# williamyang1991/VToonify

Hardware: AMD Instinct MI355X
Metric: frames/sec at 1024x1024 VToonify-D inference (higher is better)
Workload: dtype bf16

## Files before the change

### vtoonify_amd/csrc/conv_igemm.hip

```cpp
#include <stdlib.h>
#include <utility>

#include "vt_common.hpp"

namespace {

#ifdef VT_EMU
typedef emu_f32x4 f32x4;
#else
typedef float f32x4 __attribute__((ext_vector_type(4)));
typedef __bf16 bf16x8_t __attribute__((ext_vector_type(8)));
#endif

static inline int slab_ld(int cout_total) { return (cout_total + 31) / 32 * 32; }
constexpr int64_t VT_TICKET_BYTES = 16384;

struct ConvArgs {
    const void* src0;
    const void* src1;
    const void* wgt;
    const float* bias;
    const float* slope_vec;
    const void* rgb_w;
    const float* rgb_bias;
// ... 1378 lines not shown
        }
        if (rgbf && p.rgb_resid) {
#pragma unroll
            for (int j = 0; j < 3; ++j) rsd[j] = p.rgb_resid[o_rgb + (int64_t)j * HoWo];
        }
        f32x4 acc[TM][TN];
#pragma unroll
        for (int a = 0; a < TM; ++a)
#pragma unroll
            for (int b = 0; b < TN; ++b) acc[a][b] = f32x4{0.f, 0.f, 0.f, 0.f};
        const unsigned char* sa = smem + buf * A_BYTES;
#pragma unroll
        for (int t = 0; t < 9; ++t) {
            const int ky = t / 3, kx = t - ky * 3;
            u128 fa[TM];
#pragma unroll
            for (int a = 0; a < TM; ++a) {
                const int pr = (wm * TM + a + ky) * PW + kx + l15;
                fa[a] = ld128(sa + pr * 64 + ((q ^ swz(pr)) << 4));
            }
#pragma unroll
            for (int a = 0; a < TM; ++a)
#pragma unroll
                for (int b = 0; b < TN; ++b) Mma<T>::run(acc[a][b], wreg[t][b], fa[a]);
            vt_sched_fence();
        }
        {
            const float ga = p.gain_alpha;
            f32x4 racc = f32x4{0.f, 0.f, 0.f, 0.f};
#pragma unroll
            for (int a = 0; a < TM; ++a) {
                const int m = rowmap(wm * (TM * 16) + a * 16 + l15);
                float f[8];
#pragma unroll
                for (int b = 0; b < TN; ++b) {
#pragma unroll
                    for (int i = 0; i < 4; ++i) {
                        float v = acc[a][b][i] + bvr[b][i];
                        if (p.act == VT_ACT_LRELU) v = (v > 0.0f) ? v : v * p.slope;
                        f[4 * b + i] = v * ga;
                    }
                }
                const u128 fpk = pack16<bf16_t>(f);
                if (rgbf) {
                    const bool mine = (l15 >> 2) == a;
                    u128 wa;
                    wa.x = mine ? rwf.x : 0u, wa.y = mine ? rwf.y : 0u, wa.z = mine ? rwf.z : 0u, wa.w = mine ? rwf.w : 0u;
                    Mma<bf16_t>::run(racc, wa, fpk);
                }
                if (m >= 0 && !p.rgb_only) st128((bf16_t*)p.out + (int64_t)m * p.ld_out + cg + q * 8, fpk);
            }
            if (rgbf) {
                const float rr[3] = {racc[0], racc[1], racc[2]};
                if (m_rgb >= 0) {
                    p.rgb_out[o_rgb] = rr[0] + rb0 + rsd[0];
                    p.rgb_out[o_rgb + HoWo] = rr[1] + rb1 + rsd[1];
                    p.rgb_out[o_rgb + 2 * (int64_t)HoWo] = rr[2] + rb2 + rsd[2];
                }
            }
        }
        vt_lds_barrier();
        buf = buf + 1 == NBUF ? 0 : buf + 1;
    }
}

template <int... I, typename F>
__device__ __forceinline__ void vt_static_for_impl(std::integer_sequence<int, I...>, F&& f) {
    (f(std::integral_constant<int, I>{}), ...);
}
template <int N, typename F>
__device__ __forceinline__ void vt_static_for(F&& f) {
    vt_static_for_impl(std::make_integer_sequence<int, N>{}, static_cast<F&&>(f));
}

#include "conv_fullk.hpp"
#include "conv_fullkw.hpp"
#include "conv_upblur.hpp"
static int device_cus();
#include "conv_upblur_rows.hpp"
#include "conv_upblur_flat.hpp"
#include "conv_thin.hpp"
#include "conv_patch_pipe.hpp"
#include "conv_patch_chunk.hpp"
#include "conv_patch_s2.hpp"
#include "conv_patch_resident.hpp"
#include "conv_patch_persist.hpp"

__device__ __forceinline__ int slab_col4(const ConvArgs& p, int n) {
    return p.slab_perm ? (n & ~31) + ((n >> 2) & 1) * 16 + ((n >> 3) & 3) * 4 : n;
}

__global__ void __launch_bounds__(256) conv_splitk_reduce_kernel(const ConvArgs p) {
    const int nv = p.ldp / 8;
    const int64_t total = (int64_t)p.M * nv;
    const int64_t slab = (int64_t)p.M * p.ldp;
    const float ga = p.gain_alpha * (p.alpha_dev ? p.alpha_dev[0] : 1.0f);
    const int HoWo = p.Ho * p.Wo;
    for (int64_t idx = (int64_t)blockIdx.x * 256 + threadIdx.x; idx < total; idx += (int64_t)gridDim.x * 256) {
        int m, v8;
        if (p.out_layout == VT_OUT_NHWC) {
            m = (int)(idx / nv);
            v8 = (int)(idx - (int64_t)m * nv);
        } else {
            v8 = (int)(idx / p.M);
            m = (int)(idx - (int64_t)v8 * p.M);
        }
        const int n = v8 * 8;
        if (n >= p.coutT) continue;
        const int c0 = slab_col4(p, n);
        const int dc = slab_col4(p, n + 4) - c0;
        const float* src = p.partial + (int64_t)m * p.ldp + c0;
        float f[8];
        unpack16<float>(ld128(src), f);
        unpack16<float>(ld128(src + dc), f + 4);
        constexpr int SG = 8;
        for (int s0 = 1; s0 < p.splitk; s0 += SG) {
            float g[SG][8];
#pragma unroll
            for (int k = 0; k < SG; ++k) {
                const int s = (s0 + k < p.splitk) ? s0 + k : 0;
                unpack16<float>(ld128(src + s * slab), g[k]);
                unpack16<float>(ld128(src + s * slab + dc), g[k] + 4);
            }
#pragma unroll
            for (int k = 0; k < SG; ++k) {
                if (s0 + k < p.splitk) {
#pragma unroll
                    for (int i = 0; i < 8; ++i) f[i] += g[k][i];
                }
            }
        }
        {
            float bv8[8], sv8[8];
            int co8[8];
#pragma unroll
            for (int i = 0; i < 8; ++i) {
                const int nc = (n + i < p.coutT) ? n + i : 0;
                co8[i] = (p.phases > 1) ? nc % p.cout : nc;
                bv8[i] = 0.0f;
                sv8[i] = p.slope;
            }
            if (p.bias) {
#pragma unroll
                for (int i = 0; i < 8; ++i) bv8[i] = p.bias[co8[i]];
            }
            if (p.slope_vec) {
#pragma unroll
                for (int i = 0; i < 8; ++i) sv8[i] = p.slope_vec[co8[i]];
            }
#pragma unroll
            for (int i = 0; i < 8; ++i) {
                const bool okc = n + i < p.coutT;
                f[i] = conv_finish(p, f[i], okc ? bv8[i] : 0.0f, ga, okc ? sv8[i] : p.slope);
            }
        }
        if (p.out_layout == VT_OUT_NHWC) {
            store_nhwc8(p, m, n, f);
        } else {
            float* o = (float*)p.out;
            const float* rs = (const float*)p.resid;
            const int img = m / HoWo;
            const int rem = m - img * HoWo;
            for (int i = 0; i < 8 && n + i < p.coutT; ++i) {
                const int64_t off = ((int64_t)img * p.cout + n + i) * HoWo + rem;
                o[off] = post_act(p, f[i] + (rs ? p.beta * rs[off] : 0.0f));
            }
// ... 131 lines not shown
    constexpr int ESZ = (int)sizeof(T);
    constexpr int BK = 8 * (16 / ESZ);
    if (a.force_generic || a.transposed || a.in_scale) return false;
    if (a.c0 % BK != 0 || a.c1 % BK != 0) return false;
    const int64_t lim = ((int64_t)1 << 31) - 4096;
    const int64_t px = (int64_t)a.N * a.H * a.W;
    const int64_t b0 = ((int64_t)a.pad * a.W + a.pad) * a.ld0 * ESZ;
    const int64_t b1 = ((int64_t)a.pad * a.W + a.pad) * a.ld1 * ESZ;
    const int64_t n0 = px * a.ld0 * ESZ + b0, n1 = px * a.ld1 * ESZ + b1;
    const int64_t nw = (int64_t)a.coutT * a.K * ESZ;
    const int64_t tapmax = ((int64_t)(a.taps / a.kw - 1) * a.dil * a.W + (int64_t)(a.kw - 1) * a.dil);
    if (n0 + tapmax * a.ld0 * ESZ >= lim || n1 + tapmax * a.ld1 * ESZ >= lim || nw >= lim) return false;
    g.nrec0 = (uint32_t)n0;
    g.nrec1 = (uint32_t)n1;
    g.nrecw = (uint32_t)nw;
    g.bias0 = (uint32_t)b0;
    g.bias1 = (uint32_t)b1;
    return true;
}

static bool in_launch_rule(const ConvArgs& a, int64_t ntile) {
    if (a.phase != 0 || ntile * 4 > VT_TICKET_BYTES) return false;
    const char* e = getenv("VT_SPLITK_IN_LAUNCH");
    return e && e[0] == '1';
}
static void split_mode(ConvArgs& args) {
    if (args.splitk <= 1 || !in_launch_rule(args, (int64_t)args.tiles_m * args.tiles_n)) args.tickets = nullptr;
}

template <typename T, int BM, int BN, int WM, int WN>
int launch_cfg(const ConvArgs& a, vt_stream stream) {
    constexpr int BK = 8 * (16 / (int)sizeof(T));
    ConvArgs args = a;
    args.slab_perm = ((BN / WN / 16) % 2 == 0) ? 1 : 0;
    args.tiles_n = vt_cdiv(a.coutT, BN);
    args.tiles_m = vt_cdiv(a.M, BM);
    const int nk = vt_cdiv(a.K, BK);
    if (args.splitk > 1) {
        args.kps = vt_cdiv(nk, args.splitk);
        args.splitk = vt_cdiv(nk, args.kps);
    }
    if (args.splitk <= 1) {
        args.splitk = 1;
        args.kps = nk;
    }
    split_mode(args);
    const int64_t tiles = (int64_t)vt_cdiv(a.M, BM) * args.tiles_n * args.splitk;
    if (tiles >= ((int64_t)1 << 31)) {
        vt_set_error("vt_conv2d: too many tiles");
        return VT_ERR_ARG;
    }
    GldsArgs g;
    if (args.phase == 2) {
    } else if (glds_eligible<T>(args, g)) {
        if (args.splitk == 1 && args.tiles_n > 1 &&
            (int64_t)a.N * a.H * a.W * a.cin > (int64_t)a.coutT * a.K)
            args.blk_pm = -1;
        constexpr int STAGE = ((BM + 31) / 32 + (BN + 31) / 32) * 32 * 128;
        constexpr int NST = STAGE * 4 <= 80 * 1024 ? 4 : STAGE * 3 <= 80 * 1024 ? 3 : 2;
        bool done = false;
        if constexpr (sizeof(T) == 4 && !is_x3<T>::value) {
            if (a.x3) {
                auto k = conv_igemm_glds_kernel<f32x3_t, BM, BN, WM, WN, NST>;
                VT_LAUNCH(k, dim3((unsigned)tiles), dim3(256), stream, args, g);
                done = true;
            }
        }
        if (!done) {
            auto k = conv_igemm_glds_kernel<T, BM, BN, WM, WN, NST>;
            VT_LAUNCH(k, dim3((unsigned)tiles), dim3(256), stream, args, g);
        }
    } else {
        auto k = conv_igemm_kernel<T, BM, BN, WM, WN>;
        VT_LAUNCH(k, dim3((unsigned)tiles), dim3(256), stream, args);
    }
    int rc = vt_check_launch("vt_conv2d");
    if (rc != VT_OK || args.splitk == 1 || args.tickets || args.phase == 1) return rc;
    return launch_reduce<T>(args, stream);
}

struct TilePlan {
    int kind;
    int bm, bn, splitk;
};

template <typename T>
static bool patch_eligible(const ConvArgs& a, GldsArgs& g) {
    constexpr int ESZ = (int)sizeof(T);
    constexpr int BK = 8 * (16 / ESZ);
    if (a.force_generic || a.transposed || a.in_scale) return false;
    if (a.taps != 9 || a.kw != 3 || a.stride != 1 || a.pad != a.dil) return false;
    if (a.dil != 1 && a.dil != 2 && a.dil != 4) return false;
    if (a.Ho != a.H || a.Wo != a.W) return false;
    if (a.c0 % BK != 0 || a.c1 % BK != 0) return false;
    const int64_t lim = ((int64_t)1 << 31) - 4096;
    const int64_t px = (int64_t)a.N * a.H * a.W;
    const int64_t n0 = px * a.ld0 * ESZ, n1 = px * a.ld1 * ESZ, nw = (int64_t)a.coutT * a.K * ESZ;
    if (n0 >= lim || n1 >= lim || nw >= lim) return false;
    g.nrec0 = (uint32_t)n0;
    g.nrec1 = (uint32_t)n1;
    g.nrecw = (uint32_t)nw;
    g.bias0 = g.bias1 = 0;
    return true;
}

template <typename T>
static bool up_eligible(const ConvArgs& a, GldsArgs& g) {
    constexpr int ESZ = (int)sizeof(T);
    constexpr int BK = 8 * (16 / ESZ);
    if (a.force_generic || !a.transposed || a.in_scale || a.rgb_w || a.stats_part || a.tile_stats || a.in_tile_stats) return false;
    if (a.taps != 9 || a.kw != 3 || a.stride != 2 || a.pad != 0 || a.pad_x != 0 || a.dil != 1 || a.phases != 1) return false;
    if (a.Ho != 2 * a.H + 1 || a.Wo != 2 * a.W + 1 || a.c1 != 0 || a.c0 % BK != 0 || a.coutT % 8 != 0) return false;
    if (a.out_layout != VT_OUT_NHWC) return false;
    const int64_t lim = ((int64_t)1 << 31) - 4096;
    const int64_t n0 = (int64_t)a.N * a.H * a.W * a.ld0 * ESZ, nw = (int64_t)a.coutT * a.K * ESZ;
    if (n0 >= lim || nw >= lim) return false;
    g.nrec0 = (uint32_t)n0;
    g.nrec1 = 0;
    g.nrecw = (uint32_t)nw;
    g.bias0 = g.bias1 = 0;
    return true;
}

template <typename T>
static bool c32_eligible(const ConvArgs& a, GldsArgs& g) {
    if (sizeof(T) != 2 || a.force_generic || a.transposed || a.in_scale) return false;
    if (a.taps != 9 || a.kw != 3 || a.stride != 1 || a.pad != 1 || a.dil != 1) return false;
    if (a.c0 != 32 || a.c1 != 0 || a.cout % 32 != 0 || a.cout > 256 || a.phases != 1 || a.Ho != a.H || a.Wo != a.W) return false;
    if (a.cout != 32 && (a.rgb_w || a.rgb_only)) return false;
    if (a.splitk > 1) return false;
    if (a.out_layout != VT_OUT_NHWC || a.out_f32 || !a.vec_store || a.resid || a.slope_vec || a.alpha_dev || a.post_relu) return false;
    if (a.act != VT_ACT_NONE && a.act != VT_ACT_LRELU) return false;
    const int64_t n0 = (int64_t)a.N * a.H * a.W * a.ld0 * 2;
    if (n0 >= (((int64_t)1 << 31) - 4096)) return false;
    g.nrec0 = (uint32_t)n0;
    g.nrec1 = g.nrecw = g.bias0 = g.bias1 = 0;
    return true;
}

static bool batch_exact() {
    const char* be = getenv("VT_BATCH_EXACT");
    return be && be[0] == '1';
}

static int device_cus() {
#ifdef VT_EMU
    return 256;
#else
    static int cus[16] = {0};
    int dev = 0;
    if (hipGetDevice(&dev) != hipSuccess || dev < 0 || dev >= 16) return 256;
    if (!cus[dev]) {
        int n = 0;
        cus[dev] = (hipDeviceGetAttribute(&n, hipDeviceAttributeMultiprocessorCount, dev) == hipSuccess && n > 0) ? n : 256;
    }
    return cus[dev];
#endif
}
static int patchw_wgs() {
    const char* e = getenv("VT_PATCHW_WGS");
    return e && atoi(e) > 0 ? atoi(e) : device_cus();
}

template <typename T>
static TilePlan choose_plan(const ConvArgs& a, int hint, int64_t ws_floats_avail) {
    constexpr int BK = 8 * (16 / (int)sizeof(T));
    constexpr int wg_target = 256;
    TilePlan t;
    t.kind = 0;
    t.bm = t.bn = 0;
    t.splitk = 0;
    if (a.up_fir) {
        t.kind = 5;
        t.bm = 20 * 28;
        const int64_t tiles = (int64_t)vt_cdiv(2 * a.H, 20) * vt_cdiv(2 * a.W, 28);
        t.bn = (hint % 1000 == 16 || (hint % 1000 != 32 && a.N * tiles * vt_cdiv(a.coutT, 32) < 256 && a.coutT >= 32)) ? 16 : 32;
        t.splitk = 1;
        return t;
    }
    const int hp = (hint / 100000000) % 10;
    const int hs = (hint / 1000000) % 100, hbm = (hint / 1000) % 1000, hbn = hint % 1000;
    {
        GldsArgs gu;
        if (hp != 2 && hbm == 0 && hs == 0 && a.coutT >= 64 && a.cin >= 128 && up_eligible<T>(a, gu)) {
            t.kind = 1;
            t.bm = 256, t.bn = 64;
            t.splitk = 1;
            return t;
        }
    }
    {
        if ((hp == 6 || (hp == 0 && hbm == 0 && hs == 0)) && thin_eligible<T>(a)) {
            t.kind = 6;
            t.bm = thin16_wanted(a) ? TH16 * TH16 : TH_TW * TH_TW;
            t.bn = a.taps * a.coutT > 16 ? 32 : 16;
            t.splitk = 1;
            return t;
        }
    }
    const int m1 = a.Ho * a.Wo;
    auto tiles = [&](int m, int n) { return (int64_t)vt_cdiv(m1, m) * vt_cdiv(a.coutT, n); };
    auto ptiles = [&](int th, int n) {
        return (int64_t)vt_cdiv(a.Ho, th) * vt_cdiv(a.Wo, 16) * vt_cdiv(a.coutT, n);
    };
    GldsArgs g;
    if constexpr (sizeof(T) == 2) {
        GldsArgs gs;
        if ((hp == 7 || (hp == 0 && hbm == 0 && hs == 0 && (batch_exact() ? 1 : a.N) * ptiles(16, 64) >= 128)) &&
            patchs2_eligible<T>(a, gs)) {
            t.kind = 7;
            t.bm = 256, t.bn = (hbn == 32 || (hbn != 64 && (batch_exact() ? 1 : a.N) * ptiles(16, 64) < 256)) ? 32 : 64;
            t.splitk = 1;
            return t;
        }
    }
    if (hp != 2 && hbm == 0 && c32_eligible<T>(a, g)) {
        t.kind = 3;
        t.bm = 256;
        t.bn = 32;
        t.splitk = 1;
        return t;
    }
    {
        FullkArgs fg;
        const bool hinted = hp == 4;
        if (hp != 2 && (hbm == 0 || hinted) && fullk_eligible<T>(a, a.wstream, fg)) {
            const int64_t wgs = (int64_t)a.dil * a.dil * fg.tiles_y * fg.tiles_x * vt_cdiv(a.coutT, FK_BN);
            constexpr int fk_max_wgs = 1024;
            const bool batch_patch = !hinted && hbm == 0 && hp == 0 && a.N > 1 && a.dil == 1 && a.coutT >= 128 && !a.tile_stats &&
                                     !a.in_tile_stats && !a.stats_part && (int64_t)a.N * ptiles(16, 128) >= 256 &&
                                     !batch_exact() && patch_eligible<T>(a, g);
            if (batch_patch) {
                t.kind = 1;
                t.bm = 256, t.bn = 128;
                t.splitk = 1;
                return t;
            }
            const char* ppe = getenv("VT_PATCH_PIPE");
            const bool dil_ok = a.dil == 1 || (a.dil == 2 && !(ppe && ppe[0] == '0') && !a.x3);
            const bool batch_patch32 = sizeof(T) == 2 && !hinted && hbm == 0 && hp == 0 && a.N > 1 && dil_ok && m1 <= 2304 &&
                                       a.coutT >= 128 && !a.tile_stats && !a.in_tile_stats && !a.stats_part &&
                                       (int64_t)a.N * ptiles(16, 32) >= 256 && !batch_exact() && patch_eligible<T>(a, g);
            if (batch_patch32) {
                t.kind = 1;
                t.bm = 256, t.bn = 32;
                t.splitk = 1;
                return t;
            }
            if (hinted || (a.coutT >= 128 && wgs <= fk_max_wgs)) {
                t.kind = 4;
                t.bm = FK_TH * FK_TW;
                t.bn = FK_BN;
                t.splitk = 1;
                int fkw_min_g = 2;
                {
                    const char* e = getenv("VT_FULLKW");
                    const char* m = getenv("VT_FULLKW_MIN_G");
                    if (m && atoi(m) > 0) fkw_min_g = atoi(m);
                    if (e && e[0] == '0') fkw_min_g = 1 << 30;
                }
                FullkwArgs wg;
                if (fullkw_eligible<T>(a, a.wstream, wg)) {
                    const int G = fullkw_group(a.N, wg.groups_per_img, vt_cdiv(a.coutT, FK_BN));
                    if (G >= fkw_min_g) t.kind = 8, t.bm = FK_TH * FK_TW * (G > 8 ? 8 : G);
                }
                return t;
            }
        }
    }
    const bool can_patch = hp != 2 && hp != 4 && patch_eligible<T>(a, g);
    int units = 0;
    if (hbm > 0 && hp != 4) {
        t.kind = hp == 1 ? 1 : 0;
        t.bm = hbm;
        t.bn = hbn;
        t.splitk = hs;
        if (t.kind == 1 && !can_patch) t.kind = 0, t.bm = 128, t.bn = hbn >= 64 ? hbn : 64;
    } else if (can_patch) {
        t.kind = 1;
        const int units_p = a.cin / BK;
        if (a.dil == 1 && a.coutT <= 16) {
            t.bm = 128, t.bn = 16;
        } else if (a.dil == 1 && a.coutT >= 128 && ptiles(16, 128) >= 192) {
            t.bm = 256, t.bn = 128;
        } else if (a.dil == 1 && a.coutT >= 128 && (int64_t)a.N * ptiles(16, 128) >= 256 &&
                   ((ptiles(8, 128) >= 192 && ptiles(8, 64) >= 384 && !a.rgb_w) || !batch_exact())) {
            t.bm = 256, t.bn = 128;
            t.splitk = 1;
        } else if (a.dil == 1 && a.coutT == 64 && ptiles(16, 64) >= 192) {
            t.bm = 256, t.bn = 64;
        } else if (a.coutT >= 128 && ptiles(8, 128) < 192 &&
                   (a.dil == 1 || ptiles(8, 128) * units_p <= 1024)) {
            t.bm = 128, t.bn = 128;
            int64_t sk = (wg_target + ptiles(8, 128) - 1) / ptiles(8, 128);
            if (sk > units_p || a.dil != 1) sk = units_p;
            if (sk > 32) sk = 32;
            t.splitk = (int)sk;
            const int64_t need_full = (int64_t)units_p * a.M * slab_ld(a.coutT);
            if (a.dil != 1 && (sk != units_p || (units_p > 1 && (!a.partial || need_full > ws_floats_avail))))
                t.kind = 0, t.bm = 0, t.splitk = 0;
        } else if (a.dil == 1 && a.coutT >= 64) {
            t.bm = 128, t.bn = 64;
        } else {
            t.kind = 0;
        }
    }
    if (t.kind == 0 && t.bm == 0) {
        t.bn = a.coutT <= 16 ? 16 : a.coutT <= 32 ? 32 : a.coutT <= 64 ? 64 : 128;
        t.bm = 128;
        if (t.bn == 128) {
            if (tiles(128, 128) < 512) {
                t.bm = 64;
                if (tiles(64, 128) < 512 && tiles(64, 64) >= 128) t.bn = 64;
            }
        } else if (t.bn == 64) {
            if (tiles(128, 64) < 512) t.bm = 64;
        }
    }
    int64_t ntiles;
    if (t.kind == 1) {
        units = a.cin / BK;
        ntiles = ptiles(t.bm / 16, t.bn);
    } else {
        units = vt_cdiv(a.K, BK);
        ntiles = tiles(t.bm, t.bn);
    }
    if (t.splitk == 0) {
        t.splitk = 1;
        const int min_units = t.kind == 1 ? 1 : 2;
        const int64_t enough = (t.kind == 1 && t.bm == 256 ? 192 : 384) * wg_target / 256;
        if (ntiles < enough && units >= 2 * min_units) {
            int64_t sk = (2 * wg_target + ntiles - 1) / ntiles;
            if (sk > units / min_units) sk = units / min_units;
            if (sk > 32) sk = 32;
            t.splitk = (int)sk;
        }
    }
    if (t.splitk > units) t.splitk = units;
    if (t.splitk > 1) {
        const int64_t need = (int64_t)t.splitk * a.M * slab_ld(a.coutT);
        if (!a.partial || need > ws_floats_avail) t.splitk = 1;
    }
    if (t.splitk < 1) t.splitk = 1;
    const int per = vt_cdiv(units, t.splitk);
    t.splitk = vt_cdiv(units, per);
    return t;
}

template <typename T, int TH, int BN, int WM, int WN, int DIL, int NSTB, int ABUF>
int launch_patch(const ConvArgs& a, const GldsArgs& g, vt_stream stream) {
    constexpr int BK = 8 * (16 / (int)sizeof(T));
    ConvArgs args = a;
    args.slab_perm = ((BN / WN / 16) % 2 == 0) ? 1 : 0;
    args.tiles_n = vt_cdiv(a.coutT, BN);
    args.tiles_m = a.N * vt_cdiv(a.Ho, TH) * vt_cdiv(a.Wo, 16);
    const int units = a.cin / BK;
    args.kps = vt_cdiv(units, args.splitk);
    args.splitk = vt_cdiv(units, args.kps);
    split_mode(args);
    const int64_t blocks = (int64_t)args.tiles_m * args.tiles_n * args.splitk;
// ... 52 lines not shown
    args.blk_pm = args.blk_cn = 0;
    if (args.splitk != 1 || blocks < 8 || blocks % 8 != 0) return;
    const int per = (int)(blocks / 8);
    int64_t best = -1;
    for (int cn = 1; cn <= args.tiles_n; ++cn) {
        if (args.tiles_n % cn != 0 || per % cn != 0) continue;
        const int pm = per / cn;
        if (pm < 1 || args.tiles_m % pm != 0) continue;
        if ((int64_t)(args.tiles_m / pm) * (args.tiles_n / cn) != 8) continue;
        const int64_t cost = pm * patch_bytes + cn * wtile_bytes;
        if (best < 0 || cost < best) best = cost, args.blk_pm = pm, args.blk_cn = cn;
    }
}

template <typename T, int TH, int BN, int WM, int WN, int NSTB = 4, int UP = 0, int DIL = 1>
int launch_patchp(const ConvArgs& a, const GldsArgs& g, vt_stream stream) {
    constexpr int BK = 8 * (16 / (int)sizeof(T));
    ConvArgs args = a;
    args.slab_perm = ((BN / WN / 16) % 2 == 0) ? 1 : 0;
    args.tiles_n = vt_cdiv(a.coutT, BN);
    args.tiles_m = UP ? a.N * vt_cdiv(a.H + 1, TH) * vt_cdiv(a.W + 1, 16) : a.N * vt_cdiv(a.Ho, TH) * vt_cdiv(a.Wo, 16);
    const int units = a.cin / BK;
    args.kps = vt_cdiv(units, args.splitk);
    args.splitk = vt_cdiv(units, args.kps);
    split_mode(args);
    const int64_t blocks = (int64_t)args.tiles_m * args.tiles_n * args.splitk;
    if (blocks >= ((int64_t)1 << 31)) {
        vt_set_error("vt_conv2d: too many tiles");
        return VT_ERR_ARG;
    }
    if (UP == 0)
        xcd_block(args, blocks, (int64_t)(TH + 2 * DIL) * (16 + 2 * DIL) * a.cin * (int)sizeof(T), (int64_t)BN * a.K * (int)sizeof(T));
    if (args.phase != 2) {
        bool done = false;
        if constexpr (UP == 0 && (BN / WN / 16) % 2 == 0) {
            if (args.splitk == 1 && conv_lean<T>(args)) {
                auto k = conv_patchp_kernel<T, TH, BN, WM, WN, NSTB, UP, 1, DIL>;
                VT_LAUNCH(k, dim3((unsigned)blocks), dim3(WM * WN * 64), stream, args, g);
                done = true;
            }
        }
        if (!done) {
            auto k = conv_patchp_kernel<T, TH, BN, WM, WN, NSTB, UP, 0, DIL>;
            VT_LAUNCH(k, dim3((unsigned)blocks), dim3(WM * WN * 64), stream, args, g);
        }
    }
    int rc = vt_check_launch("vt_conv2d(patch, pipelined)");
    if (rc != VT_OK || args.splitk == 1 || args.tickets || args.phase == 1) return rc;
    return launch_reduce<T>(args, stream);
}

template <typename T, int DIL = 1>
int launch_patchc(const ConvArgs& a, const GldsArgs& g, vt_stream stream) {
    constexpr int TH = 16, BN = 32, WM = 8, WN = 1;
    constexpr int BK = 8 * (16 / (int)sizeof(T));
    ConvArgs args = a;
    args.slab_perm = ((BN / WN / 16) % 2 == 0) ? 1 : 0;
    args.tiles_n = vt_cdiv(a.coutT, BN);
    args.tiles_m = a.N * DIL * DIL * vt_cdiv(vt_cdiv(a.Ho, DIL), TH) * vt_cdiv(vt_cdiv(a.Wo, DIL), 16);
    const int units = a.cin / BK;
    args.kps = vt_cdiv(units, args.splitk);
    args.splitk = vt_cdiv(units, args.kps);
    split_mode(args);
    const int64_t blocks = (int64_t)args.tiles_m * args.tiles_n * args.splitk;
    if (blocks >= ((int64_t)1 << 31)) {
        vt_set_error("vt_conv2d: too many tiles");
        return VT_ERR_ARG;
    }
    xcd_block(args, blocks, (int64_t)(TH + 2) * (16 + 2) * a.cin * (int)sizeof(T), (int64_t)BN * a.K * (int)sizeof(T));
    if (args.phase != 2) {
        if (args.splitk == 1 && conv_lean<T>(args)) {
            auto k = conv_patchc_kernel<T, TH, BN, WM, WN, 1, DIL>;
            VT_LAUNCH(k, dim3((unsigned)blocks), dim3(WM * WN * 64), stream, args, g);
        } else {
            auto k = conv_patchc_kernel<T, TH, BN, WM, WN, 0, DIL>;
            VT_LAUNCH(k, dim3((unsigned)blocks), dim3(WM * WN * 64), stream, args, g);
        }
    }
    int rc = vt_check_launch("vt_conv2d(patch, chunk barriers)");
    if (rc != VT_OK || args.splitk == 1 || args.tickets || args.phase == 1) return rc;
    return launch_reduce<T>(args, stream);
}

template <typename T, int TH, int BN>
int launch_patchw(const ConvArgs& a, const GldsArgs& g, vt_stream stream) {
    ConvArgs args = a;
    args.slab_perm = ((BN / 16) % 2 == 0) ? 1 : 0;
    args.tiles_n = 1;
    args.tiles_m = a.N * vt_cdiv(a.Ho, TH) * vt_cdiv(a.Wo, 16);
    args.kps = 1;
    args.splitk = 1;
    split_mode(args);
    int wgs = patchw_wgs();
    if (wgs > args.tiles_m) wgs = args.tiles_m;
    if (wgs >= 8) wgs &= ~7;
    auto k = conv_patchw_kernel<T, TH, BN>;
    VT_LAUNCH(k, dim3((unsigned)wgs), dim3(512), stream, args, g);
    return vt_check_launch("vt_conv2d(patch, weights resident)");
}

template <typename T>
int launch_c32(const ConvArgs& a, const GldsArgs& g, vt_stream stream) {
    ConvArgs args = a;
    args.slab_perm = 0;
    args.splitk = 1;
    args.tiles_n = 1;
    args.tiles_m = a.N * vt_cdiv(a.Ho, 16) * vt_cdiv(a.Wo, 16);
    const int groups = a.cout / 32;
    const int per_group = 512 / groups > 0 ? 512 / groups : 1;
    int blocks = args.tiles_m < per_group ? args.tiles_m : per_group;
    if (const char* e = getenv("VT_C32_BLOCKS")) {
        const int v = atoi(e);
        if (v > 0 && v < blocks) blocks = v;
    }
#ifdef VT_EMU
    auto k = conv3x3_c32_kernel<bf16_t>;
#else
    auto k = conv3x3_c32_kernel<bf16_t>;
#endif
    (void)sizeof(T);
    VT_LAUNCH(k, dim3((unsigned)blocks, (unsigned)groups), dim3(256), stream, args, g);
    return vt_check_launch("vt_conv2d(c32)");
}

template <typename T>
int dispatch(const ConvArgs& a0, int hint, int64_t ws_floats, vt_stream stream) {
    ConvArgs a = a0;
    a.force_generic = hint >= 1000000000 || a.pad_x != a.pad;
    const TilePlan t = choose_plan<T>(a, hint % 1000000000, ws_floats);
    a.splitk = t.splitk;
    a.ldp = slab_ld(a.coutT);
    if (a.rgb_w && (t.bn < a.coutT || t.splitk > 1)) {
        vt_set_error("vt_conv2d: fused ToRGB needs all %d output channels in one tile (plan %dx%d, split %d)",
                     a.coutT, t.bm, t.bn, t.splitk);
        return VT_ERR_UNSUPPORTED;
    }
    if (a.in_absdiff && t.kind != 6) {
        vt_set_error("vt_conv2d: in_absdiff needs the thin-output kernel (plan kind %d)", t.kind);
        return VT_ERR_UNSUPPORTED;
    }
    if (a.rgb_only && t.kind != 3) {
        vt_set_error("vt_conv2d: rgb_only needs the persistent 32 -> 32 kernel (plan kind %d)", t.kind);
        return VT_ERR_UNSUPPORTED;
    }
    if (t.kind == 5) {
        const int chunks = a.cin / (8 * (16 / (int)sizeof(T)));
        const char* de = getenv("VT_UPBLUR_DB");
        const int64_t wgs_all = (int64_t)a.N * vt_cdiv(2 * a.H, 20) * vt_cdiv(2 * a.W, 28) * vt_cdiv(a.coutT, t.bn);
        const bool db = de ? chunks >= atoi(de) : (chunks >= 4 && (t.bn == 16 || wgs_all <= 768));
        if constexpr (sizeof(T) == 2) {
            if (uprows_wanted<T>(a)) return launch_uprows<T>(a, stream);
            if (upflat_wanted<T>(a)) return launch_upflat<T>(a, stream);
        }
        if constexpr (sizeof(T) == 2) {
            const char* p8 = getenv("VT_UPBLUR_P8");
            const int64_t tiles8 = (int64_t)a.N * vt_cdiv(2 * a.H, 28) * vt_cdiv(2 * a.W, 28) * vt_cdiv(a.coutT, 32);
            const bool on = p8 ? p8[0] == '1' : tiles8 >= 1024;
            if (on && t.bn == 32 && chunks == 1) return launch_upblur<T, 32, 16, 0, 1, 0, 8>(a, stream);
        }
        {
            const char* te = getenv("VT_UPBLUR_TALL");
            const int64_t tall_min = te ? atoll(te) : 448;
            const int64_t wgs_tall = (int64_t)a.N * vt_cdiv(2 * a.H, 44) * vt_cdiv(2 * a.W, 28) * vt_cdiv(a.coutT, 32);
            if constexpr (sizeof(T) == 2) {
                if (t.bn == 32 && !db && chunks >= (te ? 2 : 4) && tall_min > 0 && wgs_tall >= tall_min)
                    return launch_upblur<T, 32, 24, 0, 0, 0, 8>(a, stream);
// ... 12 lines not shown
        return VT_ERR_UNSUPPORTED;
    }
    if (a.in_tile_stats && a.c1 != 0) {
        vt_set_error("vt_conv2d: in_tile_stats (AdaIN prologue) supports a single source");
        return VT_ERR_UNSUPPORTED;
    }
    if (t.kind == 6) return launch_thin<T>(a, stream);
    if (t.kind == 7) {
        GldsArgs gs;
        if constexpr (sizeof(T) == 2) {
            if (patchs2_eligible<T>(a, gs)) return t.bn == 32 ? launch_patchs2<T, 32>(a, gs, stream) : launch_patchs2<T, 64>(a, gs, stream);
        }
        vt_set_error("vt_conv2d: stride-2 patch kernel requested for an ineligible convolution");
        return VT_ERR_UNSUPPORTED;
    }
    if (t.kind == 8) {
        FullkwArgs wg;
        if (!fullkw_eligible<T>(a, a.wstream, wg)) {
            vt_set_error("vt_conv2d: weight-stationary whole-K kernel requested for an ineligible convolution");
            return VT_ERR_UNSUPPORTED;
        }
        return launch_fullkw<T>(a, wg, t.bm / (FK_TH * FK_TW), stream);
    }
    if (t.kind == 4) {
        FullkArgs fg;
        if (!fullk_eligible<T>(a, a.wstream, fg)) {
            vt_set_error("vt_conv2d: whole-K kernel requested for an ineligible convolution");
            return VT_ERR_UNSUPPORTED;
        }
        return launch_fullk<T>(a, fg, stream);
    }
    if (t.kind == 3) {
        GldsArgs g;
        if (!c32_eligible<T>(a, g)) {
            vt_set_error("vt_conv2d: c32 kernel requested for an ineligible convolution");
            return VT_ERR_UNSUPPORTED;
        }
        return launch_c32<T>(a, g, stream);
    }
    if (t.kind == 1 && a.transposed) {
        GldsArgs g;
        if (!up_eligible<T>(a, g)) {
            vt_set_error("vt_conv2d: transposed patch plan requested for an ineligible convolution");
            return VT_ERR_UNSUPPORTED;
        }
        return launch_patchp<T, 16, 64, 4, 2, 8, 1>(a, g, stream);
    }
    if (t.kind == 1) {
        GldsArgs g;
        if (!patch_eligible<T>(a, g)) {
            vt_set_error("vt_conv2d: patch kernel requested for an ineligible convolution");
            return VT_ERR_UNSUPPORTED;
        }
        const int units = a.cin / (8 * (16 / (int)sizeof(T)));
        const bool one_chunk = vt_cdiv(units, a.splitk) == 1;
#define VT_PATCH(TH_, BN_, WM_, WN_, DIL_, NSTB_, ABUF_, COND_) \
    if (t.bm == TH_ * 16 && t.bn == BN_ && a.dil == DIL_ && (COND_))  \
        return launch_patch<T, TH_, BN_, WM_, WN_, DIL_, NSTB_, ABUF_>(a, g, stream);
        {
            const char* e = getenv("VT_PATCH_PIPE");
            const bool pipe = !(e && e[0] == '0') && !a.x3;
            if constexpr (sizeof(T) == 2) {
                const bool lean = a.coutT == 64 && a.phases == 1 && a.out_layout == VT_OUT_NHWC && !a.out_f32 && a.vec_store &&
                                  a.ld_out % 8 == 0 && !a.resid && !a.slope_vec && !a.alpha_dev && !a.post_relu && !a.stats_part &&
                                  (a.act == VT_ACT_NONE || a.act == VT_ACT_LRELU) &&
                                  (int64_t)a.N * a.Ho * a.Wo * a.ld_out * 2 < (((int64_t)1 << 31) - 4096) &&
                                  (int64_t)a.N * a.Ho * a.Wo * 12 < (((int64_t)1 << 31) - 4096);
                if (pipe && !(e && e[0] == '1') && a.dil == 1 && t.bm == 256 && t.bn == 64 && units == 1 && lean && !a.src1 &&
                    a.splitk <= 1 &&
                    (int64_t)(batch_exact() ? 1 : a.N) * vt_cdiv(a.Ho, 16) * vt_cdiv(a.Wo, 16) >= 2 * patchw_wgs())
                    return launch_patchw<T, 16, 64>(a, g, stream);
            }
            if constexpr (sizeof(T) == 2) {
                if (pipe && !(e && e[0] == '1') && a.dil == 1 && t.bm == 256 && (t.bn == 128 || t.bn == 64) && a.splitk <= 1 &&
                    conv_lean<T>(a) && vt_cdiv(a.coutT, t.bn) * t.bn * 8 <= PQ_TAB_BYTES &&
                    (int64_t)a.N * vt_cdiv(a.Ho, 16) * vt_cdiv(a.Wo, 16) * vt_cdiv(a.coutT, t.bn) > patchw_wgs()) {
                    if (t.bn == 128) return launch_patchq<T, 16, 128, 4, 2, 4>(a, g, stream);
                    return launch_patchq<T, 16, 64, 4, 2, 4>(a, g, stream);
                }
            }
            if (pipe && a.dil == 1 && t.bm == 256 && t.bn == 128) return launch_patchp<T, 16, 128, 4, 2>(a, g, stream);
            if (pipe && a.dil == 1 && t.bm == 256 && t.bn == 64) return launch_patchp<T, 16, 64, 4, 2, 4>(a, g, stream);
            if constexpr (sizeof(T) == 2) {
                if (pipe && !(e && e[0] == '1') && a.dil == 1 && t.bm == 256 && t.bn == 32) return launch_patchc<T>(a, g, stream);
                if (pipe && !(e && e[0] == '1') && a.dil == 2 && t.bm == 256 && t.bn == 32 && !a.stats_part)
                    return launch_patchc<T, 2>(a, g, stream);
            }
            if (pipe && a.dil == 1 && t.bm == 256 && t.bn == 32) return launch_patchp<T, 16, 32, 8, 1, 8>(a, g, stream);
            if (pipe && a.dil == 2 && t.bm == 256 && t.bn == 32) return launch_patchp<T, 16, 32, 8, 1, 6, 0, 2>(a, g, stream);
        }
        VT_PATCH(16, 128, 4, 2, 1, 3, 2, true)
        VT_PATCH(16, 64, 4, 2, 1, 3, 2, true)
        VT_PATCH(8, 64, 2, 2, 1, 3, 2, true)
        VT_PATCH(8, 16, 4, 1, 1, 3, 2, true)
        VT_PATCH(8, 128, 2, 2, 1, 6, 1, one_chunk)
        VT_PATCH(8, 128, 2, 2, 2, 6, 1, one_chunk)
        VT_PATCH(8, 128, 2, 2, 4, 6, 1, one_chunk)
        VT_PATCH(8, 128, 2, 2, 1, 6, 2, !one_chunk)
#undef VT_PATCH
        vt_set_error("vt_conv2d: no compiled patch tile %dx%d dil %d", t.bm, t.bn, a.dil);
        return VT_ERR_UNSUPPORTED;
    }
    const int bm = t.bm, bn = t.bn;
#define VT_CFG(M_, N_, WM_, WN_) \
    if (bm == M_ && bn == N_) return launch_cfg<T, M_, N_, WM_, WN_>(a, stream);
    VT_CFG(128, 128, 2, 2)
    VT_CFG(128, 64, 2, 2)
    VT_CFG(128, 32, 4, 1)
    VT_CFG(128, 16, 4, 1)
    VT_CFG(64, 64, 2, 2)
    VT_CFG(64, 128, 2, 2)
    VT_CFG(32, 64, 2, 2)
#undef VT_CFG
    vt_set_error("vt_conv2d: no compiled tile %dx%d", bm, bn);
    return VT_ERR_UNSUPPORTED;
}

}

static int fill_args(const vt_conv_desc* d, ConvArgs& a) {
    VT_REQUIRE(d, "vt_conv2d: null descriptor");
    VT_REQUIRE(d->src0 && d->weight && d->out, "vt_conv2d: null tensor");
    VT_REQUIRE(d->dtype == VT_F32 || d->dtype == VT_BF16 || d->dtype == VT_F32X3, "vt_conv2d: dtype must be fp32, bf16 or f32x3");
    const int cdt = d->dtype == VT_F32X3 ? VT_F32 : d->dtype;
    VT_REQUIRE(d->c0 > 0 && d->c0 % 8 == 0 && d->c1 >= 0 && d->c1 % 8 == 0,
               "vt_conv2d: channel counts must be multiples of 8 (got %d,%d)", d->c0, d->c1);
    VT_REQUIRE(d->c1 == 0 || d->src1, "vt_conv2d: c1 > 0 but src1 is null");
    VT_REQUIRE(d->ld0 >= d->c0 && (d->c1 == 0 || d->ld1 >= d->c1), "vt_conv2d: pixel stride < channels");
    const int esz = cdt == VT_F32 ? 4 : 2;
    VT_REQUIRE(((uintptr_t)d->src0 % 16 == 0) && ((int64_t)d->ld0 * esz % 16 == 0) &&
                   ((uintptr_t)d->weight % 16 == 0),
               "vt_conv2d: src0/weight must be 16-byte aligned with 16-byte pixel stride");
    VT_REQUIRE(d->c1 == 0 || (((uintptr_t)d->src1 % 16 == 0) && ((int64_t)d->ld1 * esz % 16 == 0)),
               "vt_conv2d: src1 must be 16-byte aligned with 16-byte pixel stride");
    VT_REQUIRE(d->n > 0 && d->h > 0 && d->w > 0 && d->out_h > 0 && d->out_w > 0, "vt_conv2d: bad sizes");
    VT_REQUIRE(d->kh > 0 && d->kw > 0 && d->stride > 0 && d->dil > 0 && d->cout > 0, "vt_conv2d: bad conv params");
    VT_REQUIRE(d->phases == 1 || d->phases == 4, "vt_conv2d: phases must be 1 or 4");
    VT_REQUIRE(d->phases == 1 || (d->cout % 8 == 0 && d->out_layout == VT_OUT_NHWC && !d->transposed),
               "vt_conv2d: polyphase form needs cout %% 8 == 0 and NHWC output");
    VT_REQUIRE(d->out_layout == VT_OUT_NHWC || d->out_dtype == VT_F32, "vt_conv2d: NCHW output is fp32 only");
    VT_REQUIRE(d->out_dtype == VT_F32 || d->out_dtype == VT_BF16, "vt_conv2d: bad out dtype");
    VT_REQUIRE((int64_t)d->n * d->h * d->w < ((int64_t)1 << 31) &&
                   (int64_t)d->n * d->out_h * d->out_w * (d->phases == 4 ? 4 : 1) < ((int64_t)1 << 31),
               "vt_conv2d: tensor too large for 32-bit pixel indices");

    VT_REQUIRE(!d->stats_part || (d->phases == 1 && d->out_layout == VT_OUT_NHWC && d->out_dtype == cdt &&
                                  d->cout % 8 == 0 && (cdt == VT_BF16 || cdt == VT_F32)),
               "vt_conv2d: stats_part needs phases == 1, NHWC output in the compute dtype, cout %% 8 == 0");
    VT_REQUIRE(!d->post_relu || !d->rgb_weight, "vt_conv2d: post_relu cannot be combined with the fused ToRGB");
    VT_REQUIRE(!d->rgb_weight || (d->rgb_out && d->phases == 1 && d->out_layout == VT_OUT_NHWC && !d->transposed),
               "vt_conv2d: fused ToRGB needs rgb_out, phases == 1 and NHWC output");
    memset(&a, 0, sizeof(a));
    a.src0 = d->src0;
    a.src1 = d->src1;
    a.wgt = d->weight;
    a.bias = d->bias;
    a.slope_vec = d->slope_vec;
    a.rgb_w = d->rgb_weight;
    a.rgb_bias = d->rgb_bias;
    a.rgb_resid = d->rgb_resid;
    a.rgb_out = d->rgb_out;
    a.stats_part = (StatRec*)d->stats_part;
    a.x3 = d->dtype == VT_F32X3 ? 1 : 0;
    a.alpha_dev = d->alpha_dev;
    a.post_relu = d->post_relu ? 1 : 0;
    a.wstream = d->weight_stream;
// ... 175 lines not shown
```

Baseline: 1683.

## Add intra-workgroup K-split patch conv kernel for 256x32 trunk tiles

Adds a new 512-thread patch convolution kernel that splits each BK chunk's reduction across two wave groups, with four wave pairs each owning four output rows. Partial accumulators are then summed through LDS before the shared epilogue. It is selected by default for bf16 256x32 patch tiles (dil 1 or 2) on the batched patch32 path, replacing the chunk-barrier kernel there. The aim is more waves per tile for latency hiding and MFMA throughput on thin-output trunk convs, at the cost of an extra LDS exchange and barrier in the epilogue.

New measurement: 1686, median of 6. About the same (+0.2%).

```diff
diff --git a/vtoonify_amd/csrc/conv_igemm.hip b/vtoonify_amd/csrc/conv_igemm.hip
--- a/vtoonify_amd/csrc/conv_igemm.hip
+++ b/vtoonify_amd/csrc/conv_igemm.hip
@@ -1484,6 +1484,7 @@
 #include "conv_thin.hpp"
 #include "conv_patch_pipe.hpp"
 #include "conv_patch_chunk.hpp"
+#include "conv_patch_ksplit.hpp"
 #include "conv_patch_s2.hpp"
 #include "conv_patch_resident.hpp"
 #include "conv_patch_persist.hpp"
@@ -1781,7 +1782,13 @@
 struct TilePlan {
     int kind;
     int bm, bn, splitk;
+    int ks;
 };
+
+template <typename T>
+static bool ksplit_ok(const ConvArgs& a, int bm, int bn) {
+    return sizeof(T) == 2 && !a.x3 && bm == 256 && bn == 32 && (a.dil == 1 || (a.dil == 2 && !a.stats_part));
+}
 
 template <typename T>
 static bool patch_eligible(const ConvArgs& a, GldsArgs& g) {
@@ -1869,6 +1876,7 @@
     t.kind = 0;
     t.bm = t.bn = 0;
     t.splitk = 0;
+    t.ks = 0;
     if (a.up_fir) {
         t.kind = 5;
         t.bm = 20 * 28;
@@ -1944,6 +1952,7 @@
                 t.kind = 1;
                 t.bm = 256, t.bn = 32;
                 t.splitk = 1;
+                t.ks = !(ppe && ppe[0] >= '0' && ppe[0] <= '2') && ksplit_ok<T>(a, t.bm, t.bn);
                 return t;
             }
             if (hinted || (a.coutT >= 128 && wgs <= fk_max_wgs)) {
@@ -1970,11 +1979,12 @@
     const bool can_patch = hp != 2 && hp != 4 && patch_eligible<T>(a, g);
     int units = 0;
     if (hbm > 0 && hp != 4) {
-        t.kind = hp == 1 ? 1 : 0;
+        t.kind = (hp == 1 || hp == 3) ? 1 : 0;
         t.bm = hbm;
         t.bn = hbn;
         t.splitk = hs;
         if (t.kind == 1 && !can_patch) t.kind = 0, t.bm = 128, t.bn = hbn >= 64 ? hbn : 64;
+        t.ks = t.kind == 1 && hp == 3 && ksplit_ok<T>(a, t.bm, t.bn);
     } else if (can_patch) {
         t.kind = 1;
         const int units_p = a.cin / BK;
@@ -2193,6 +2203,38 @@
     return launch_reduce<T>(args, stream);
 }
 
+template <typename T, int DIL = 1>
+int launch_patchk(const ConvArgs& a, const GldsArgs& g, vt_stream stream) {
+    constexpr int TH = 16, BN = 32;
+    constexpr int BK = 8 * (16 / (int)sizeof(T));
+    ConvArgs args = a;
+    args.slab_perm = 1;
+    args.tiles_n = vt_cdiv(a.coutT, BN);
+    args.tiles_m = a.N * DIL * DIL * vt_cdiv(vt_cdiv(a.Ho, DIL), TH) * vt_cdiv(vt_cdiv(a.Wo, DIL), 16);
+    const int units = a.cin / BK;
+    args.kps = vt_cdiv(units, args.splitk);
+    args.splitk = vt_cdiv(units, args.kps);
+    split_mode(args);
+    const int64_t blocks = (int64_t)args.tiles_m * args.tiles_n * args.splitk;
+    if (blocks >= ((int64_t)1 << 31)) {
+        vt_set_error("vt_conv2d: too many tiles");
+        return VT_ERR_ARG;
+    }
+    xcd_block(args, blocks, (int64_t)(TH + 2) * (16 + 2) * a.cin * (int)sizeof(T), (int64_t)BN * a.K * (int)sizeof(T));
+    if (args.phase != 2) {
+        if (args.splitk == 1 && conv_lean<T>(args)) {
+            auto k = conv_patchk_kernel<T, 1, DIL>;
+            VT_LAUNCH(k, dim3((unsigned)blocks), dim3(512), stream, args, g);
+        } else {
+            auto k = conv_patchk_kernel<T, 0, DIL>;
+            VT_LAUNCH(k, dim3((unsigned)blocks), dim3(512), stream, args, g);
+        }
+    }
+    int rc = vt_check_launch("vt_conv2d(patch, K-split trunk)");
+    if (rc != VT_OK || args.splitk == 1 || args.tickets || args.phase == 1) return rc;
+    return launch_reduce<T>(args, stream);
+}
+
 template <typename T, int TH, int BN>
 int launch_patchw(const ConvArgs& a, const GldsArgs& g, vt_stream stream) {
     ConvArgs args = a;
@@ -2371,6 +2413,8 @@
             if (pipe && a.dil == 1 && t.bm == 256 && t.bn == 128) return launch_patchp<T, 16, 128, 4, 2>(a, g, stream);
             if (pipe && a.dil == 1 && t.bm == 256 && t.bn == 64) return launch_patchp<T, 16, 64, 4, 2, 4>(a, g, stream);
             if constexpr (sizeof(T) == 2) {
+                if (t.ks && a.dil == 1) return launch_patchk<T>(a, g, stream);
+                if (t.ks && a.dil == 2) return launch_patchk<T, 2>(a, g, stream);
                 if (pipe && !(e && e[0] == '1') && a.dil == 1 && t.bm == 256 && t.bn == 32) return launch_patchc<T>(a, g, stream);
                 if (pipe && !(e && e[0] == '1') && a.dil == 2 && t.bm == 256 && t.bn == 32 && !a.stats_part)
                     return launch_patchc<T, 2>(a, g, stream);
diff --git a/vtoonify_amd/csrc/conv_patch_ksplit.hpp b/vtoonify_amd/csrc/conv_patch_ksplit.hpp
--- /dev/null
+++ b/vtoonify_amd/csrc/conv_patch_ksplit.hpp
@@ -0,0 +1,173 @@
+#pragma once
+
+template <typename T, int EPI = 0, int DIL = 1>
+__global__ void __launch_bounds__(512)
+conv_patchk_kernel(const ConvArgs p, const GldsArgs g) {
+    constexpr int TH = 16, TW = 16, BN = 32;
+    constexpr int NW = 8;
+    constexpr int BM = TH * TW;
+    constexpr int ESZ = (int)sizeof(T);
+    constexpr int VEC = 16 / ESZ;
+    constexpr int BK = 8 * VEC;
+    constexpr int TN = BN / 16;
+    constexpr int RW = 4;
+    constexpr int PH = TH + 2, PW = TW + 2, PROWS = PH * PW;
+    constexpr int NPA = (PROWS + 7) / 8, NPB = BN / 8;
+    constexpr int PA = (NPA + NW - 1) / NW;
+    constexpr int LB = (9 * NPB + NW - 1) / NW;
+    constexpr int A_BYTES = NPA * 1024, B_BYTES = NPB * 1024;
+    constexpr int C_BYTES = A_BYTES + 9 * B_BYTES;
+    static_assert(ESZ == 2, "bf16 MFMA fragments");
+    static_assert(NW % NPB == 0, "a wave's weight pieces are the same rows of every slab it loads");
+    static_assert(2 * C_BYTES <= 160 * 1024, "LDS budget: two whole chunks");
+    static_assert(PA + LB < 64, "vmcnt is 6 bits");
+
+    __shared__ __attribute__((aligned(1024))) unsigned char smem[2 * C_BYTES];
+
+    const int tid = threadIdx.x;
+    const int lane = tid & 63;
+    const int wave = vt_uniform(tid >> 6) & (NW - 1);
+    const int pw = wave >> 1, kg = wave & 1;
+    int tile_m, tile_n, split;
+    decode_block_2d(p, tile_m, tile_n, split);
+    const int tiles_x = ((p.Wo + DIL - 1) / DIL + TW - 1) / TW;
+    const int tiles_y = ((p.Ho + DIL - 1) / DIL + TH - 1) / TH;
+    const int per_img = DIL * DIL * tiles_x * tiles_y;
+    const int img = tile_m / per_img;
+    int trem = tile_m - img * per_img;
+    const int sub = trem / (tiles_x * tiles_y);
+    trem -= sub * (tiles_x * tiles_y);
+    const int sy = sub / DIL, sx = sub - sy * DIL;
+    const int y0 = (trem / tiles_x) * TH, x0 = (trem % tiles_x) * TW;
+    const int n0 = tile_n * BN;
+
+    const int lrow = lane >> 3;
+    const int jj = (lane & 7) ^ lrow;
+    uint32_t pa0[PA], pa1[PA];
+#pragma unroll
+    for (int i = 0; i < PA; ++i) {
+        const int pr = (i * NW + wave) * 8 + lrow;
+        const int py = pr / PW, px = pr - py * PW;
+        const int iy = (y0 - 1 + py) * DIL + sy, ix = (x0 - 1 + px) * DIL + sx;
+        const bool in = pr < PROWS && (unsigned)iy < (unsigned)p.H && (unsigned)ix < (unsigned)p.W;
+        const uint32_t pix = (uint32_t)((img * p.H + iy) * p.W + ix);
+        pa0[i] = in ? pix * (uint32_t)(p.ld0 * ESZ) + jj * 16 : GLDS_OOB;
+        pa1[i] = in ? pix * (uint32_t)(p.ld1 * ESZ) + jj * 16 : GLDS_OOB;
+    }
+    const int wsub = wave % NPB;
+    uint32_t woff;
+    {
+        const int row = wsub * 8 + lrow;
+        const int n = n0 + tile_row_channel<true>(row);
+        woff = (n < p.coutT) ? (uint32_t)n * (uint32_t)(p.K * ESZ) + jj * 16 : GLDS_OOB;
+    }
+    const BufRsrc r0 = vt_make_rsrc(p.src0, g.nrec0);
+    const BufRsrc r1 = vt_make_rsrc(p.src1 ? p.src1 : p.src0, p.src1 ? g.nrec1 : 0u);
+    const BufRsrc rw = vt_make_rsrc(p.wgt, g.nrecw);
+
+    const int nchunks = p.cin / BK;
+    const int ch0 = split * p.kps;
+    const int ch1 = (ch0 + p.kps < nchunks) ? ch0 + p.kps : nchunks;
+
+    auto issue_chunk = [&](int chunk, int coff) {
+        const int kc = chunk * BK;
+        const bool s1 = kc >= p.c0;
+        const uint32_t so = (uint32_t)((s1 ? kc - p.c0 : kc) * ESZ);
+#pragma unroll
+        for (int i = 0; i < PA; ++i)
+            if ((i + 1) * NW <= NPA || i * NW + wave < NPA)
+                vt_glds16(s1 ? r1 : r0, smem + coff + (i * NW + wave) * 1024, s1 ? pa1[i] : pa0[i], so);
+#pragma unroll
+        for (int i = 0; i < LB; ++i) {
+            const int w = i * NW + wave;
+            const int tap = w / NPB;
+            if ((i + 1) * NW <= 9 * NPB || w < 9 * NPB)
+                vt_glds16(rw, smem + coff + A_BYTES + w * 1024, woff, (uint32_t)((tap * p.cin + kc) * ESZ));
+        }
+    };
+
+    f32x4 acc[RW][TN];
+#pragma unroll
+    for (int a = 0; a < RW; ++a)
+#pragma unroll
+        for (int b = 0; b < TN; ++b) acc[a][b] = f32x4{0.f, 0.f, 0.f, 0.f};
+
+    const int q = lane >> 4, l15 = lane & 15, l7 = lane & 7;
+    const int rbase = pw * RW * PW + l15;
+    uint32_t aswz[8];
+#pragma unroll
+    for (int cm = 0; cm < 8; ++cm) aswz[cm] = (uint32_t)(rbase * 128 + (((kg * 4 + q) ^ ((rbase + cm) & 7)) << 4));
+    const uint32_t bfix = (uint32_t)(A_BYTES + l15 * 128 + (((kg * 4 + q) ^ l7) << 4));
+
+    u128 fa[2][RW + 2], fb[2][3][TN];
+    auto read_frags = [&](auto dxc, u128 (&xa)[RW + 2], u128 (&xb)[3][TN], int coff) {
+        constexpr int DX = decltype(dxc)::value;
+        auto rd_a = [&](int r) {
+            const int rowc = r * PW + DX;
+            xa[r] = ld128(smem + coff + aswz[rowc & 7] + rowc * 128);
+        };
+        auto rd_b = [&](int dy) {
+#pragma unroll
+            for (int b = 0; b < TN; ++b) xb[dy][b] = ld128(smem + coff + (dy * 3 + DX) * B_BYTES + bfix + b * 2048);
+        };
+        rd_b(0);
+#pragma unroll
+        for (int r = 0; r < RW; ++r) rd_a(r);
+        rd_b(1);
+        rd_a(RW);
+        rd_b(2);
+        rd_a(RW + 1);
+    };
+    auto mma_step = [&](const u128 (&xa)[RW + 2], const u128 (&xb)[3][TN]) {
+#pragma unroll
+        for (int dy = 0; dy < 3; ++dy)
+#pragma unroll
+            for (int a = 0; a < RW; ++a)
+#pragma unroll
+                for (int b = 0; b < TN; ++b) Mma<T>::run(acc[a][b], xb[dy][b], xa[a + dy]);
+    };
+    EpiTables<TN> etab;
+    epi_tables<TN, true>(p, n0, q, etab);
+
+    issue_chunk(ch0, 0);
+    vt_glds_wait();
+    vt_lds_barrier();
+
+    int coff = 0;
+    for (int chunk = ch0; chunk < ch1; ++chunk) {
+        if (chunk + 1 < ch1) issue_chunk(chunk + 1, coff ^ C_BYTES);
+        read_frags(std::integral_constant<int, 0>{}, fa[0], fb[0], coff);
+        vt_static_for<3>([&](auto dxc) {
+            constexpr int dx = decltype(dxc)::value;
+            vt_sched_fence();
+            if constexpr (dx + 1 < 3) read_frags(std::integral_constant<int, dx + 1>{}, fa[(dx + 1) & 1], fb[(dx + 1) & 1], coff);
+            mma_step(fa[dx & 1], fb[dx & 1]);
+        });
+        vt_sched_fence();
+        vt_glds_wait();
+        vt_lds_barrier();
+        coff ^= C_BYTES;
+    }
+
+    {
+        static_assert(NW * RW * TN * 1024 <= 2 * C_BYTES, "K-group exchange fits the chunk buffers");
+        unsigned char* mine = smem + wave * (RW * TN * 1024) + lane * 16;
+#pragma unroll
+        for (int a = 0; a < RW; ++a)
+#pragma unroll
+            for (int b = 0; b < TN; ++b) *reinterpret_cast<f32x4*>(mine + (a * TN + b) * 1024) = acc[a][b];
+        __syncthreads();
+        const unsigned char* h0 = smem + (2 * pw) * (RW * TN * 1024) + (2 * kg) * (TN * 1024) + lane * 16;
+        const unsigned char* h1 = h0 + RW * TN * 1024;
+        f32x4 fin[2][TN];
+#pragma unroll
+        for (int a = 0; a < 2; ++a)
+#pragma unroll
+            for (int b = 0; b < TN; ++b)
+                fin[a][b] = *reinterpret_cast<const f32x4*>(h0 + (a * TN + b) * 1024) +
+                            *reinterpret_cast<const f32x4*>(h1 + (a * TN + b) * 1024);
+        __syncthreads();
+        conv_epilogue<T, BM, BN, NW, 1, EPI>(p, fin, smem, SubImageRows<TW, DIL>{img, y0, x0, sy, sx, p.Ho, p.Wo}, n0, split,
+                                             tile_n * p.tiles_m + tile_m, etab);
+    }
+}
```
